# Deam0on/deepEMIA

Hardware: AMD Instinct MI355X
Metric: EM tiles/s (2048x2048, R101-FPN) (higher is better)
Workload: dtype f16x2

## Files before the change

### deepemia_amd/csrc/conv_p32.hip

```cpp
#include <utility>
#include "common.h"
#ifndef P32_ABLATE
#define P32_ABLATE 0
#endif

#ifndef P32_HEAD_DIRECT
#define P32_HEAD_DIRECT 1
#endif
#ifndef P32_SINGLE
#define P32_SINGLE 0
#endif
#ifndef P32_DEV_TILES
#define P32_DEV_TILES 0
#endif
#ifndef P32_ST_AUX
#define P32_ST_AUX 0
#endif
#ifndef P32_RES_AUX
#define P32_RES_AUX 0
#endif
#ifndef P32_A_NT
#define P32_A_NT 0
#endif
#ifndef P32_FRAG_PIPE
// ... 92 lines not shown
#pragma unroll
        for (int r = 0; r < 16; ++r)
            e[((r & 3) + 8 * (r >> 2) + 4 * (lane >> 5)) * EF + j * 32 + (lane & 31)] = row[j][r];
}
template <int TN, int EF>
__device__ __forceinline__ void write_acc16(const f32x4 (&r0)[2 * TN], const f32x4 (&r1)[2 * TN], float* e, int lane) {
#pragma unroll
    for (int j = 0; j < 2 * TN; ++j)
#pragma unroll
        for (int r = 0; r < 4; ++r) {
            e[(4 * (lane >> 4) + r) * EF + j * 16 + (lane & 15)] = r0[j][r];
            e[(16 + 4 * (lane >> 4) + r) * EF + j * 16 + (lane & 15)] = r1[j][r];
        }
}

__device__ __forceinline__ float uniform(float v) { return __int_as_float(__builtin_amdgcn_readfirstlane(__float_as_int(v))); }

struct GroupScales {
    int g0, b1, b2;
    float post0, post1, post2, resi0, resi1, resi2, sout0, sout1, sout2;
};

__device__ __forceinline__ void load_group_scale(const ConvQ& p, int gi, bool planes_out, float& post, float& resi, float& sout) {
    gi = min(gi, p.groups - 1);
    const float amax_in = p.in_meta[2 * gi], s_in = p.in_meta[2 * gi + 1];
    float amax_res = 0.f, s_res = 1.f;
    if (p.res_mode != DEMIA_RES_NONE) { amax_res = p.res_meta[2 * gi]; s_res = p.res_meta[2 * gi + 1]; }
    post = uniform(1.0f / s_in);
    resi = uniform(p.res_mode != DEMIA_RES_NONE ? 1.0f / s_res : 0.f);
    sout = uniform(planes_out ? plane_scale(amax_in * p.wbound + p.bbound + amax_res) : 1.f);
}

__device__ __forceinline__ GroupScales load_group_scales(const ConvQ& p, int m0, bool planes_out) {
    GroupScales gs;
    gs.g0 = (m0 + p.row0) / p.group_rows;
    gs.b1 = (gs.g0 + 1) * p.group_rows - p.row0;
    gs.b2 = gs.b1 + p.group_rows;
    load_group_scale(p, gs.g0, planes_out, gs.post0, gs.resi0, gs.sout0);
    load_group_scale(p, gs.g0 + 1, planes_out, gs.post1, gs.resi1, gs.sout1);
    load_group_scale(p, gs.g0 + 2, planes_out, gs.post2, gs.resi2, gs.sout2);
    return gs;
}

__device__ __forceinline__ float scale_shift(float acc, float post, float sc, float bs) { return (acc * post) * sc + bs; }
__device__ __forceinline__ void planes_item(const float4 x0, const float4 x1, float post, float res_inv, float s_out, const float (&sc)[8],
                                            const float (&bs)[8], const f16x8 ch, const f16x8 cl, float act_lo, bool sigmoid_on,
                                            f16x8& h, f16x8& l, float& vm) {
    typedef float f32x2 __attribute__((ext_vector_type(2)));
    f32x2 v2[4] = {{x0.x, x0.y}, {x0.z, x0.w}, {x1.x, x1.y}, {x1.z, x1.w}};
    float v[8];
#pragma unroll
    for (int q = 0; q < 4; ++q) {
        const f32x2 scq = {sc[2 * q], sc[2 * q + 1]}, bsq = {bs[2 * q], bs[2 * q + 1]};
        const f32x2 t = (v2[q] * post) * scq + bsq;
        v[2 * q] = t.x;
        v[2 * q + 1] = t.y;
    }
#pragma unroll
    for (int q = 0; q < 8; ++q) {
        v[q] = fmaf((float)cl[q], res_inv, fmaf((float)ch[q], res_inv, v[q]));
        v[q] = fmaxf(v[q], act_lo);
    }
    if (sigmoid_on && !(P32_ABLATE & 256)) {
#pragma unroll
        for (int q = 0; q < 8; ++q) v[q] = 1.0f / (1.0f + expf(-v[q]));
    }
    vm = 0.f;
#pragma unroll
    for (int q = 0; q < 8; q += 2) {
        vm = fmaxf(vm, fmaxf(fabsf(v[q]), fabsf(v[q + 1])));
        const f32x2 y = f32x2{v[q], v[q + 1]} * s_out;
        h[q] = (_Float16)y.x;
        h[q + 1] = (_Float16)y.y;
        l[q] = (_Float16)fmaf(-(float)h[q], 1.0f, y.x);
        l[q + 1] = (_Float16)fmaf(-(float)h[q + 1], 1.0f, y.y);
    }
}

template <int WM, int WN, int TM, int TN, bool HEAD, typename WriteRow>
__device__ __forceinline__ void p32_epilogue(const ConvQ& p, const GroupScales& gs, char* smem, WriteRow&& write_tile_row, int wm, int wn, int m0, int n0) {
    constexpr int BN = WN * TN * 32;
    const int tid = threadIdx.x, lane = tid & 63;
    constexpr int EROW = BN * 4 + 16;
    constexpr int GPR = BN / 8, RSTEP = 512 / GPR, ITEMS = WM * 32 / RSTEP;
    static_assert(512 % GPR == 0 && (WM * 32) % RSTEP == 0, "epilogue split");
    constexpr int BM_ = WM * TM * 32;
    static_assert(!HEAD || BN == 256, "the fused head needs a 256-wide tile");
    const bool planes_out = !HEAD && !p.out_f32;
    const int g0 = __builtin_amdgcn_readfirstlane(gs.g0), b1 = __builtin_amdgcn_readfirstlane(gs.b1), b2 = __builtin_amdgcn_readfirstlane(gs.b2);
    const float post0 = uniform(gs.post0), post1 = uniform(gs.post1), post2 = uniform(gs.post2);
    const float resi0 = uniform(gs.resi0), resi1 = uniform(gs.resi1), resi2 = uniform(gs.resi2);
    const float sout0 = uniform(gs.sout0), sout1 = uniform(gs.sout1), sout2 = uniform(gs.sout2);
    if (planes_out && n0 == 0 && tid == 0) {
#pragma unroll
        for (int d = 0; d < 3; ++d) {
            const int first = d == 0 ? g0 * p.group_rows - p.row0 : (d == 1 ? b1 : b2);
            if (g0 + d < p.groups && first >= m0 && first < m0 + BM_ && first < p.M)
                p.out_meta[2 * (g0 + d) + 1] = d == 0 ? sout0 : (d == 1 ? sout1 : sout2);
        }
    }
    const int g = tid % GPR, r_first = tid / GPR;
    const int co = n0 + g * 8;
    float sc[8], bs[8];
#pragma unroll
    for (int q = 0; q < 8; ++q) {
        const bool ok = (co + q) < p.Cout;
        sc[q] = (p.scale && ok) ? p.scale[co + q] : 1.0f;
        bs[q] = (p.bias && ok) ? p.bias[co + q] : 0.0f;
    }
    float vmax3[3] = {0.f, 0.f, 0.f};
    constexpr int HMAX = 4;
    float hw[HMAX][8];
    constexpr bool head_on = HEAD;
    if (head_on) {
#pragma unroll
        for (int j = 0; j < HMAX; ++j)
#pragma unroll
            for (int q = 0; q < 8; ++q) hw[j][q] = j < p.head_n ? p.head_w[j * 256 + g * 8 + q] : 0.f;
    }
    const int tile_n_ = n0 / BN;
    const bool res_on = p.res_mode != DEMIA_RES_NONE, sigmoid_on = p.act == DEMIA_ACT_SIGMOID;
    const float act_lo = p.act == DEMIA_ACT_RELU ? 0.f : -INFINITY;
    const char* resb = reinterpret_cast<const char*>(p.res) + 128;
    char* outb = reinterpret_cast<char*>(p.out) + 128;
    const long cbytes = (long)p.Cout * 4;
    const int gofs = (co >> 5) * 128 + ((co & 31) >> 3) * 16;
    auto row_of = [&](int i, int k) { const int lr = r_first + k * RSTEP; return m0 + (lr >> 5) * (TM * 32) + i * 32 + (lr & 31); };
    auto res_pix = [&](int m) -> long {
        if (p.res_mode == DEMIA_RES_SAME) return m;
        const int n = m / p.HoWo;
        const int rem = m - n * p.HoWo;
        const int ho = rem / p.Wo, wo = rem - ho * p.Wo;
        const int Hr = (p.Ho + 1) >> 1, Wr = (p.Wo + 1) >> 1;
        return ((long)n * Hr + (ho >> 1)) * Wr + (wo >> 1);
    };
    f16x8 rh[ITEMS], rl[ITEMS];
    const bool has_res = p.res_mode != DEMIA_RES_NONE && co < p.Cout;
    auto load_res = [&](int i) {
#pragma unroll
        for (int k = 0; k < ITEMS; ++k) {
            const int m = row_of(i, k);
            if (has_res && m < p.M && !(P32_ABLATE & 32)) {
                const char* rp = resb + res_pix(m) * cbytes + gofs;
                rh[k] = *reinterpret_cast<const f16x8*>(rp);
                rl[k] = *reinterpret_cast<const f16x8*>(rp + 64);
            }
        }
    };
    load_res(0);
#pragma unroll
    for (int i = 0; i < TM; ++i) {
        if (i > 0) __syncthreads();
        write_tile_row(i, reinterpret_cast<float*>(smem) + (wm * 32) * (EROW / 4) + wn * TN * 32);
        __syncthreads();
        f16x8 ch[ITEMS], cl[ITEMS];
#pragma unroll
        for (int k = 0; k < ITEMS; ++k) { ch[k] = rh[k]; cl[k] = rl[k]; }
        if (i + 1 < TM) load_res(i + 1);
        if (co < p.Cout) {
#pragma unroll
            for (int k = 0; k < ITEMS; ++k) {
                const int lr = r_first + k * RSTEP;
                const int m = row_of(i, k);
                if (m >= p.M) continue;
                const float4 x0 = *reinterpret_cast<const float4*>(smem + lr * EROW + g * 32);
                const float4 x1 = *reinterpret_cast<const float4*>(smem + lr * EROW + g * 32 + 16);
                float v[8] = {x0.x, x0.y, x0.z, x0.w, x1.x, x1.y, x1.z, x1.w};
                const int gd = (m >= b1) + (m >= b2);
// ... 27 lines not shown
#pragma unroll
                        for (int j = 0; j < HMAX; ++j)
                            if (j < p.head_n) {
                                const float z = acc_h[j] + p.head_b[j];
                                o[j] = p.head_act == DEMIA_ACT_SIGMOID ? 1.0f / (1.0f + expf(-z)) : (p.head_act == DEMIA_ACT_RELU ? fmaxf(z, 0.f) : z);
                            }
                    }
                } else if (p.out_f32) {
                    float* o = reinterpret_cast<float*>(p.out) + (long)m * p.out_ld + co;
                    if (co + 8 <= p.Cout && (p.out_ld & 3) == 0) {
                        *reinterpret_cast<float4*>(o) = make_float4(v[0], v[1], v[2], v[3]);
                        *reinterpret_cast<float4*>(o + 4) = make_float4(v[4], v[5], v[6], v[7]);
                    } else {
#pragma unroll
                        for (int q = 0; q < 8; ++q)
                            if (co + q < p.Cout) o[q] = v[q];
                    }
                } else {
                    f16x8 h, l;
                    const float s_out = gd == 0 ? sout0 : (gd == 1 ? sout1 : sout2);
                    float vm = 0.f;
#pragma unroll
                    for (int q = 0; q < 8; ++q) {
                        vm = fmaxf(vm, fabsf(v[q]));
                        const float y = v[q] * s_out;
                        h[q] = (_Float16)y;
                        l[q] = (P32_SINGLE && p.zero_low) ? (_Float16)0.f : (_Float16)(y - (float)h[q]);
                    }
                    vmax3[0] = fmaxf(vmax3[0], gd == 0 ? vm : 0.f);
                    vmax3[1] = fmaxf(vmax3[1], gd == 1 ? vm : 0.f);
                    vmax3[2] = fmaxf(vmax3[2], gd == 2 ? vm : 0.f);
                    char* o = outb + (long)m * cbytes + gofs;
                    if (P32_ABLATE & 64) {
                        asm volatile("" :: "v"(h), "v"(l), "v"(o));
                    } else {
                        *reinterpret_cast<f16x8*>(o) = h;
                        *reinterpret_cast<f16x8*>(o + 64) = l;
                    }
                }
            }
        }
    }
    if (planes_out) {
#pragma unroll
        for (int d = 0; d < 3; ++d) {
            if (d > 0 && (d == 1 ? b1 : b2) >= m0 + BM_) break;
            if (g0 + d >= p.groups) break;
            float vmax = vmax3[d];
#pragma unroll
            for (int o = 32; o > 0; o >>= 1) vmax = fmaxf(vmax, __shfl_xor(vmax, o));
            float* slot = p.out_meta + 2 * (g0 + d);
            if (lane == 0 && vmax > *reinterpret_cast<volatile const float*>(slot))
                atomicMax(reinterpret_cast<unsigned int*>(slot), __float_as_uint(vmax));
        }
    }
}

struct NoHook { __device__ __forceinline__ void operator()() const {} };
template <int WM, int WN, int TM, int TN, typename WriteRow, typename Hook = NoHook>
__device__ __forceinline__ void p32_epilogue_planes(const ConvQ& p, const GroupScales& gs, char* smem, WriteRow&& write_tile_row, int wm, int wn,
                                                    int m0, int n0, bool leader = (threadIdx.x == 0), Hook&& hook = NoHook()) {
    constexpr int BM_ = WM * TM * 32;
    const int tid = threadIdx.x, lane = tid & 63;
    constexpr int LDW = TN * 32 + 4;
    constexpr int PPW = 8 / TN, RPI = 2 * PPW, ITEMS = 32 / RPI;
    static_assert(TN == 1 || TN == 2 || TN == 4, "TN");
    char* const wsm = smem + (tid >> 6) * (32 * LDW * 4);
    const int g0 = __builtin_amdgcn_readfirstlane(gs.g0), b1 = __builtin_amdgcn_readfirstlane(gs.b1), b2 = __builtin_amdgcn_readfirstlane(gs.b2);
    const float post0 = uniform(gs.post0), post1 = uniform(gs.post1), post2 = uniform(gs.post2);
    const float resi0 = uniform(gs.resi0), resi1 = uniform(gs.resi1), resi2 = uniform(gs.resi2);
    const float sout0 = uniform(gs.sout0), sout1 = uniform(gs.sout1), sout2 = uniform(gs.sout2);
    if (n0 == 0 && leader) {
#pragma unroll
        for (int d = 0; d < 3; ++d) {
            const int first = d == 0 ? g0 * p.group_rows - p.row0 : (d == 1 ? b1 : b2);
            if (g0 + d < p.groups && first >= m0 && first < m0 + BM_ && first < p.M)
                p.out_meta[2 * (g0 + d) + 1] = d == 0 ? sout0 : (d == 1 ? sout1 : sout2);
        }
    }
    const int cj = lane & 3, rs = (lane >> 2) & 1, lg = lane >> 3;
    const int line = lg % TN;
    const int r_first = (lg / TN) * 2 + rs;
    const int co = n0 + ((wn * TN + line) * 4 + cj) * 8;
    float sc[8], bs[8];
#pragma unroll
    for (int q = 0; q < 8; ++q) {
        sc[q] = p.scale ? p.scale[co + q] : 1.0f;
        bs[q] = p.bias ? p.bias[co + q] : 0.0f;
    }
    const bool sigmoid_on = p.act == DEMIA_ACT_SIGMOID;
    const float act_lo = p.act == DEMIA_ACT_RELU ? 0.f : -INFINITY;
    const bool res_on = p.res_mode != DEMIA_RES_NONE;
    const bool single = P32_SINGLE != 0 && p.zero_low != 0;
    const __amdgpu_buffer_rsrc_t rs_out = __builtin_amdgcn_make_buffer_rsrc(p.out, 0, (int)p.out_bytes, 0x00020000);
    const __amdgpu_buffer_rsrc_t rs_res = __builtin_amdgcn_make_buffer_rsrc(const_cast<void*>(res_on ? p.res : p.out), 0, res_on ? (int)p.res_bytes : 0, 0x00020000);
    const unsigned cbytes = (unsigned)p.Cout * 4u;
    const unsigned lofs = 128u + (unsigned)((co >> 5) * 128 + (lane & 7) * 16);
    auto row_of = [&](int i, int k) { return m0 + wm * (TM * 32) + i * 32 + r_first + k * RPI; };
    auto res_off = [&](int m) -> unsigned {
        if (p.res_mode != DEMIA_RES_UP2 || (P32_ABLATE & 256)) return (unsigned)m * cbytes + lofs;
        const int n = m / p.HoWo;
        const int rem = m - n * p.HoWo;
        const int ho = rem / p.Wo, wo = rem - ho * p.Wo;
        const int Hr = (p.Ho + 1) >> 1, Wr = (p.Wo + 1) >> 1;
        return (unsigned)((n * Hr + (ho >> 1)) * Wr + (wo >> 1)) * cbytes + lofs;
    };
    auto from_below = [&](u32x4 own, u32x4 theirs) -> u32x4 {
        u32x4 r;
#pragma unroll
        for (int c = 0; c < 4; ++c) r[c] = (unsigned)__builtin_amdgcn_update_dpp((int)own[c], (int)theirs[c], 0x114, 0xf, 0xa, false);
        return r;
    };
    auto from_above = [&](u32x4 own, u32x4 theirs) -> u32x4 {
        u32x4 r;
#pragma unroll
        for (int c = 0; c < 4; ++c) r[c] = (unsigned)__builtin_amdgcn_update_dpp((int)own[c], (int)theirs[c], 0x104, 0xf, 0x5, false);
        return r;
    };
    u32x4 rh[ITEMS], rl[ITEMS];
    auto load_res = [&](int i) {
#pragma unroll
        for (int k = 0; k < ITEMS; ++k) {
            const int mp = row_of(i, k) - rs;
            if (P32_ABLATE & 32) { rh[k] = u32x4{0, 0, 0, 0}; rl[k] = rh[k]; continue; }
            rh[k] = __builtin_amdgcn_raw_buffer_load_b128(rs_res, res_off(mp), 0, P32_RES_AUX);
            rl[k] = __builtin_amdgcn_raw_buffer_load_b128(rs_res, res_off(mp + 1), 0, P32_RES_AUX);
        }
    };
    float vmax0 = 0.f, vmax1 = 0.f, vmax2 = 0.f;
    if (P32_ABLATE & 512) return;
    load_res(0);
#pragma unroll
    for (int i = 0; i < TM; ++i) {
        asm volatile("" ::: "memory");
        __builtin_amdgcn_wave_barrier();
        write_tile_row(i, reinterpret_cast<float*>(wsm));
        asm volatile("" ::: "memory");
        __builtin_amdgcn_wave_barrier();
        f16x8 ch[ITEMS], cl[ITEMS];
#pragma unroll
        for (int k = 0; k < ITEMS; ++k) {
            ch[k] = __builtin_bit_cast(f16x8, from_below(rh[k], rl[k]));
            cl[k] = __builtin_bit_cast(f16x8, from_above(rl[k], rh[k]));
        }
        if (i + 1 < TM) load_res(i + 1);
#pragma unroll
        for (int k = 0; k < ITEMS; ++k) {
            const int lr = r_first + k * RPI;
            const int m = row_of(i, k);
            const float4 x0 = *reinterpret_cast<const float4*>(wsm + lr * (LDW * 4) + (line * 4 + cj) * 32);
            const float4 x1 = *reinterpret_cast<const float4*>(wsm + lr * (LDW * 4) + (line * 4 + cj) * 32 + 16);
            const int gd = (m >= b1) + (m >= b2);
            const float post = gd == 0 ? post0 : (gd == 1 ? post1 : post2);
            const float res_inv = gd == 0 ? resi0 : (gd == 1 ? resi1 : resi2);
            const float s_out = gd == 0 ? sout0 : (gd == 1 ? sout1 : sout2);
            f16x8 h, l;
            float vm;
            planes_item(x0, x1, post, res_inv, s_out, sc, bs, ch[k], cl[k], act_lo, sigmoid_on, h, l, vm);
            if (single) l = f16x8{0, 0, 0, 0, 0, 0, 0, 0};
            vm = m < p.M ? vm : 0.f;
            vmax0 = fmaxf(vmax0, gd == 0 ? vm : 0.f);
            vmax1 = fmaxf(vmax1, gd == 1 ? vm : 0.f);
            vmax2 = fmaxf(vmax2, gd == 2 ? vm : 0.f);
            const u32x4 hu = __builtin_bit_cast(u32x4, h), lu = __builtin_bit_cast(u32x4, l);
            const u32x4 d0 = from_below(hu, lu);
            const u32x4 d1 = from_above(lu, hu);
            const unsigned off = (unsigned)(m - rs) * cbytes + lofs;
            if (P32_ABLATE & 64) {
                asm volatile("" :: "v"(d0), "v"(d1), "v"(off));
            } else {
                __builtin_amdgcn_raw_buffer_store_b128(d0, rs_out, off, 0, P32_ST_AUX);
                __builtin_amdgcn_raw_buffer_store_b128(d1, rs_out, off + cbytes, 0, P32_ST_AUX);
            }
            hook();
        }
    }
#pragma unroll
    for (int d = 0; d < 3; ++d) {
        if (d > 0 && (d == 1 ? b1 : b2) >= m0 + BM_) break;
        if (g0 + d >= p.groups) break;
        float vmax = d == 0 ? vmax0 : (d == 1 ? vmax1 : vmax2);
#pragma unroll
        for (int o = 32; o > 0; o >>= 1) vmax = fmaxf(vmax, __shfl_xor(vmax, o));
        float* slot = p.out_meta + 2 * (g0 + d);
        if (lane == 0 && vmax > *reinterpret_cast<volatile const float*>(slot))
            atomicMax(reinterpret_cast<unsigned int*>(slot), __float_as_uint(vmax));
    }
}

template <int WM, int WN, int TM, int TN, int HN>
__device__ __forceinline__ void p32_epilogue_head_direct(const ConvQ& p, const GroupScales& gs, char* smem, const f32x4 (&acc16)[2 * TM][2 * TN],
                                                         int wm, int wn, int m0, int n0) {
    constexpr int BM = WM * TM * 32, BN = WN * TN * 32;
    static_assert(BN == 256, "the fused head needs a 256-wide tile");
    const int tid = threadIdx.x, lane = tid & 63, c16 = lane & 15, rq = lane >> 4;
    const int b1 = __builtin_amdgcn_readfirstlane(gs.b1), b2 = __builtin_amdgcn_readfirstlane(gs.b2);
    const float post0 = uniform(gs.post0), post1 = uniform(gs.post1), post2 = uniform(gs.post2);
    float sc[2 * TN], bs[2 * TN], hw[HN][2 * TN];
#pragma unroll
    for (int jn = 0; jn < 2 * TN; ++jn) {
        const int cl = wn * TN * 32 + jn * 16 + c16;
        sc[jn] = p.scale ? p.scale[n0 + cl] : 1.0f;
        bs[jn] = p.bias ? p.bias[n0 + cl] : 0.0f;
#pragma unroll
        for (int j = 0; j < HN; ++j) hw[j][jn] = j < p.head_n ? p.head_w[j * 256 + cl] : 0.f;
    }
    const float act_lo = p.act == DEMIA_ACT_RELU ? 0.f : -INFINITY;
    float* part = reinterpret_cast<float*>(smem);
#pragma unroll
    for (int i = 0; i < 2 * TM; ++i) {
#pragma unroll
        for (int r = 0; r < 4; ++r) {
            const int row = wm * TM * 32 + i * 16 + rq * 4 + r;
            const int m = m0 + row;
            const int gd = (m >= b1) + (m >= b2);
            const float post = gd == 0 ? post0 : (gd == 1 ? post1 : post2);
            float a[HN];
#pragma unroll
            for (int j = 0; j < HN; ++j) a[j] = 0.f;
#pragma unroll
            for (int jn = 0; jn < 2 * TN; ++jn) {
                const float v = fmaxf((acc16[i][jn][r] * post) * sc[jn] + bs[jn], act_lo);
#pragma unroll
                for (int j = 0; j < HN; ++j) a[j] = fmaf(v, hw[j][jn], a[j]);
            }
#pragma unroll
            for (int j = 0; j < HN; ++j) {
                a[j] += __int_as_float(__builtin_amdgcn_update_dpp(0, __float_as_int(a[j]), 0x128, 0xf, 0xf, false));
                a[j] += __int_as_float(__builtin_amdgcn_update_dpp(0, __float_as_int(a[j]), 0x124, 0xf, 0xf, false));
                a[j] += __int_as_float(__builtin_amdgcn_update_dpp(0, __float_as_int(a[j]), 0x122, 0xf, 0xf, false));
// ... 52 lines not shown
    const int line = lg % TN;
    const int r_first = (lg / TN) * 2 + rs;
    const int cgrp = wn * TN + line;
    const int co = (cgrp * 4 + cj) * 8;
    float sc[8], bs[8];
#pragma unroll
    for (int q = 0; q < 8; ++q) {
        sc[q] = p.scale ? p.scale[co + q] : 1.0f;
        bs[q] = p.bias ? p.bias[co + q] : 0.0f;
    }
    const bool sigmoid_on = p.act == DEMIA_ACT_SIGMOID;
    const float act_lo = p.act == DEMIA_ACT_RELU ? 0.f : -INFINITY;
    const f16x8 zero8 = {0, 0, 0, 0, 0, 0, 0, 0};
    const int r16 = lane & 15, kq = lane >> 4, fsw = (r16 >> 1) & 7;
    const bool c_ok = r16 < p.hp_cout;
    const float hsc = (p.hp_scale && c_ok) ? p.hp_scale[r16] : 1.0f;
    const float hbs = (p.hp_bias && c_ok) ? p.hp_bias[r16] : 0.0f;
#pragma unroll
    for (int i = 0; i < TM; ++i) {
        asm volatile("" ::: "memory");
        __builtin_amdgcn_wave_barrier();
        write_tile_row(i, reinterpret_cast<float*>(wsm));
        asm volatile("" ::: "memory");
        __builtin_amdgcn_wave_barrier();
        f16x8 h[ITEMS], l[ITEMS];
#pragma unroll
        for (int k = 0; k < ITEMS; ++k) {
            const int lr = r_first + k * RPI;
            const int m = m0 + wm * (TM * 32) + i * 32 + lr;
            const float4 x0 = *reinterpret_cast<const float4*>(wsm + lr * (LDW * 4) + (line * 4 + cj) * 32);
            const float4 x1 = *reinterpret_cast<const float4*>(wsm + lr * (LDW * 4) + (line * 4 + cj) * 32 + 16);
            const int gd = (m >= b1) + (m >= b2);
            const float post = gd == 0 ? post0 : (gd == 1 ? post1 : post2);
            const float s_out = gd == 0 ? sout0 : (gd == 1 ? sout1 : sout2);
            float vm;
            planes_item(x0, x1, post, 0.f, s_out, sc, bs, zero8, zero8, act_lo, sigmoid_on, h[k], l[k], vm);
        }
        if (i > 0) __syncthreads();
#pragma unroll
        for (int k = 0; k < ITEMS; ++k) {
            const int R = wm * 32 + r_first + k * RPI, sw = (R >> 1) & 7;
            char* ln = img + (cgrp * ROWS + R) * 128;
            *reinterpret_cast<f16x8*>(ln + ((cj ^ sw) * 16)) = h[k];
            *reinterpret_cast<f16x8*>(ln + (((4 + cj) ^ sw) * 16)) = l[k];
        }
        if (i == 0) {
#pragma unroll
            for (int q = 0; q < 2; ++q) {
                const int c = tid + q * 512, g = c >> 7, row = (c >> 3) & 15, ck = c & 7;
                *reinterpret_cast<u32x4*>(wimg + g * 2048 + row * 128 + ((ck ^ ((row >> 1) & 7)) * 16)) = wreg[q];
            }
        }
        __syncthreads();
        if (wave < ROWS / 16) {
            f32x4 c = {0.f, 0.f, 0.f, 0.f};
#pragma unroll
            for (int g = 0; g < 8; ++g) {
                const char* ab = img + (g * ROWS + wave * 16 + r16) * 128;
                const char* bb = wimg + g * 2048 + r16 * 128;
                const f16x8 ah = *reinterpret_cast<const f16x8*>(ab + ((kq ^ fsw) * 16));
                const f16x8 al = *reinterpret_cast<const f16x8*>(ab + (((4 + kq) ^ fsw) * 16));
                const f16x8 bh = *reinterpret_cast<const f16x8*>(bb + ((kq ^ fsw) * 16));
                const f16x8 bl = *reinterpret_cast<const f16x8*>(bb + (((4 + kq) ^ fsw) * 16));
                c = __builtin_amdgcn_mfma_f32_16x16x32_f16(ah, bl, c, 0, 0, 0);
                c = __builtin_amdgcn_mfma_f32_16x16x32_f16(al, bh, c, 0, 0, 0);
                c = __builtin_amdgcn_mfma_f32_16x16x32_f16(ah, bh, c, 0, 0, 0);
            }
#pragma unroll
            for (int r = 0; r < 4; ++r) {
                const int R = wave * 16 + kq * 4 + r;
                const int m = m0 + (R >> 5) * (TM * 32) + i * 32 + (R & 31);
                const int gd = (m >= b1) + (m >= b2);
                const float ipost = gd == 0 ? ipost0 : (gd == 1 ? ipost1 : ipost2);
                const float z = fmaxf(scale_shift(c[r], ipost, hsc, hbs), -INFINITY);
                if (m < p.M && c_ok) p.head_out[(long)m * p.head_ld + r16] = z;
            }
        }
    }
}

constexpr int EPI_GENERIC = 0, EPI_PLANES = 1, EPI_HEAD = 2, EPI_HEAD_PLANES = 3;

template <int WM, int WN, int TM, int TN, bool M16 = true, int EPI = EPI_PLANES, int NST = 2, bool HK = false>
__global__ __launch_bounds__(WM * WN * 64, WM * WN == 8 ? 2 : 1) void conv_p32_kernel(const ConvQ p) {
    static_assert(NST == 2 || NST == 3, "two or three LDS stages");
    static_assert(!HK || (P32_SINGLE && M16 && NST == 2), "HK is a variant of the single-plane 16x16x32 kernel");
    static_assert(WM * WN == 8 || (WM * WN == 4 && EPI == EPI_PLANES), "eight waves, or four (planes epilogue only)");
    constexpr int NW = WM * WN;
    constexpr int BM = WM * TM * 32, BN = WN * TN * 32;
    constexpr int STAGE = (BM + BN) * 128;
    constexpr int NIA = BM / 8, NIB = BN / 8;

    extern __shared__ __attribute__((aligned(16))) char smem[];
    const int tid = threadIdx.x, lane = tid & 63;
    const int wave = __builtin_amdgcn_readfirstlane(tid >> 6);
    const int wm = wave / WN, wn = wave % WN;
    const int swz = xcd_remap(blockIdx.x, p.nwg);
    const int tile_n = swz % p.ntn, tile_m = swz / p.ntn;
    const int m0 = tile_m * BM, n0 = tile_n * BN;
#if P32_DEV_TILES
    if (p.stagger_ticks > 0) {
        const int b = blockIdx.x;
        const bool late = p.resident > 256 ? (b >= p.resident / 2 && b < p.resident) : (b < p.resident && ((b >> 3) & 1));
        if (late) {
            const unsigned long long t0 = __builtin_amdgcn_s_memrealtime();
            while (__builtin_amdgcn_s_memrealtime() - t0 < (unsigned long long)p.stagger_ticks) __builtin_amdgcn_s_sleep(32);
        }
    }
#endif

    const i32x4 rsrc_a = make_rsrc(p.in, p.in_bytes), rsrc_b = make_rsrc(p.w, p.w_bytes);
    const unsigned lds0 = (unsigned)(__SIZE_TYPE__)((lds_void*)smem);

    constexpr int QA = (NIA + NW - 1) / NW, QB = NIB / NW;
    constexpr bool A_EVEN = NIA % NW == 0;
    static_assert(NIB % NW == 0, "tile width is a multiple of 64");
    unsigned a_off[QA], a_msk[QA], b_off[QB];
#pragma unroll
    for (int q = 0; q < QA; ++q) {
        const int row = (wave + NW * q) * 8 + (lane >> 3);
        const int csw = (lane & 7) ^ ((row >> 1) & 7);
        const int m = m0 + row;
        const bool vm = m < p.M && row < BM;
        const int mm = vm ? m : 0;
        const int n = mm / p.HoWo;
        const int rem = mm - n * p.HoWo;
        const int ho = rem / p.Wo, wo = rem - ho * p.Wo;
        const int hi0 = ho * p.stride - p.pad, wi0 = wo * p.stride - p.pad;
        const long pix = ((long)n * p.H + hi0) * p.W + wi0;
        a_off[q] = (unsigned)(128 + pix * (long)(p.Cin * 4) + (HK ? (csw >> 2) * 128 + (csw & 3) * 16 : csw * 16));
        unsigned mk = 0;
        for (int t = 0, th = 0, tw = 0; t < p.taps; ++t) {
            if (vm && (unsigned)(hi0 + th) < (unsigned)p.H && (unsigned)(wi0 + tw) < (unsigned)p.W) mk |= 1u << t;
            if (++tw == p.KW) { tw = 0; ++th; }
        }
        a_msk[q] = mk;
    }
#pragma unroll
    for (int q = 0; q < QB; ++q) {
        const int row = (wave + NW * q) * 8 + (lane >> 3);
        const int csw = (lane & 7) ^ ((row >> 1) & 7);
        const int co = n0 + row;
        b_off[q] = (unsigned)(((co >> 6) * p.ksteps) * 8192 + (co & 63) * 128 + (HK ? (csw >> 2) * (p.taps * 8192) + (csw & 3) * 16 : csw * 16));
    }
    int tap = 0, kw = 0, tstep = 0;
    unsigned sdelta = 0, srow = 0, sgrp = 0;
    const bool a_nt = P32_A_NT && p.taps == 1 && p.ntn == 1;
    auto issue = [&](int st, int tp, unsigned sd, unsigned bd) {
        const unsigned sbase = __builtin_amdgcn_readfirstlane(lds0 + st * STAGE + wave * 1024);
        const bool first = bd < 2 * 8192u;
#pragma unroll
        for (int q = 0; q < QA; ++q) {
            if ((P32_ABLATE & 1) && !first) break;
            if (!A_EVEN && q == QA - 1 && wave + NW * q >= NIA) break;
            const bool ok = (a_msk[q] >> tp) & 1u;
            const unsigned vo = ok ? a_off[q] + sd : (a_off[q] & 0x70u);
            if (P32_A_NT && a_nt) dma16_nt(rsrc_a, sbase + q * (NW * 1024), vo, 0u);
            else dma16(rsrc_a, sbase + q * (NW * 1024), vo, 0u);
        }
#pragma unroll
        for (int q = 0; q < QB; ++q) {
            if ((P32_ABLATE & 2) && !first) break;
            dma16(rsrc_b, sbase + BM * 128 + q * (NW * 1024), b_off[q], bd);
        }
    };
    const unsigned pixb = (unsigned)(p.Cin * 4), rowb = (unsigned)(p.W * p.Cin * 4);
#define P32_ADVANCE()                                                                   \
    do {                                                                                \
        ++tstep;                                                                        \
        if (++tap == p.taps) { tap = 0; kw = 0; srow = 0; sgrp += HK ? 256u : 128u; sdelta = sgrp; if (HK) tstep += p.taps; } \
// ... 192 lines not shown
#pragma unroll
        for (int kk = 0; kk < 2; ++kk) {
            f16x8 bh[TN], bl[TN];
#pragma unroll
            for (int j = 0; j < TN; ++j) {
                bh[j] = *reinterpret_cast<const f16x8*>(sb + fb[kk] + j * 4096);
                bl[j] = *reinterpret_cast<const f16x8*>(sb + fb[2 + kk] + j * 4096);
            }
#pragma unroll
            for (int i = 0; i < TM; ++i) {
                const f16x8 ah = *reinterpret_cast<const f16x8*>(sb + fa[kk] + i * 4096);
                const f16x8 al = *reinterpret_cast<const f16x8*>(sb + fa[2 + kk] + i * 4096);
#pragma unroll
                for (int j = 0; j < TN; ++j) {
                    f32x16 c = acc[i][j];
                    if (P32_ABLATE & 4) {
                        asm volatile("" :: "v"(ah), "v"(al), "v"(bh[j]), "v"(bl[j]));
                        continue;
                    }
                    c = __builtin_amdgcn_mfma_f32_32x32x16_f16(ah, bl[j], c, 0, 0, 0);
                    c = __builtin_amdgcn_mfma_f32_32x32x16_f16(al, bh[j], c, 0, 0, 0);
                    c = __builtin_amdgcn_mfma_f32_32x32x16_f16(ah, bh[j], c, 0, 0, 0);
                    acc[i][j] = c;
                }
            }
        }
    };

    constexpr int N_LAST = QB + QA, N_LAST_SHORT = QB + QA - 1;
    const bool short_wave = !A_EVEN && wave + NW * (QA - 1) >= NIA;
    auto wait_all_but_last_issue = [&]() {
        if (short_wave) asm volatile("s_waitcnt vmcnt(%0)" ::"n"(N_LAST_SHORT) : "memory");
        else asm volatile("s_waitcnt vmcnt(%0)" ::"n"(N_LAST) : "memory");
    };
    issue(0, tap, sdelta, 0u);
    P32_ADVANCE();
    bool two_ahead = false;
    if (NST == 3 && p.kloop > 1 && !(P32_ABLATE & 128)) {
        issue(1, tap, sdelta, (unsigned)tstep * 8192u);
        P32_ADVANCE();
        two_ahead = true;
    }
    constexpr bool HEAD = EPI == EPI_HEAD;
    const GroupScales gs = load_group_scales(p, m0, !HEAD && !p.out_f32);
    if (two_ahead) wait_all_but_last_issue();
    else asm volatile("s_waitcnt vmcnt(0)" ::: "memory");
    __builtin_amdgcn_s_barrier();
    int st = 0;
    for (int t = 0; t < ((P32_ABLATE & 128) ? 1 : p.kloop); ++t) {
        const int st_issue = NST == 2 ? (st ^ 1) : (st == 0 ? 2 : st - 1);
        const bool more = t + NST - 1 < p.kloop;
        if (more) {
            issue(st_issue, tap, sdelta, (unsigned)tstep * 8192u);
            P32_ADVANCE();
        }
        compute(st);
        if (NST == 3 && more) {
            wait_all_but_last_issue();
            asm volatile("s_waitcnt lgkmcnt(0)\n\ts_barrier" ::: "memory");
        } else if (!BARRIER_IN_COMPUTE) {
            asm volatile("s_waitcnt vmcnt(0) lgkmcnt(0)\n\ts_barrier" ::: "memory");
        }
        st = NST == 2 ? (st ^ 1) : (st == 2 ? 0 : st + 1);
    }
#undef P32_ADVANCE

    if constexpr ((P32_ABLATE & 2048) != 0 && M16) {
#pragma unroll
        for (int i = 0; i < 2 * TM; ++i)
#pragma unroll
            for (int j = 0; j < 2 * TN; ++j) asm volatile("" :: "v"(acc16[i][j]));
        return;
    }
    if constexpr (EPI == EPI_HEAD_PLANES) {
        static_assert(M16, "the fused 1x1 layer rides on the 16x16x32 kernel");
        p32_epilogue_head_planes<WM, WN, TM, TN>(p, gs, smem, [&](int i, float* e) { write_acc16<TN, TN * 32 + 4>(acc16[2 * i], acc16[2 * i + 1], e, lane); }, wm, wn, m0);
    } else if constexpr (EPI == EPI_PLANES) {
        if constexpr (M16) {
            p32_epilogue_planes<WM, WN, TM, TN>(p, gs, smem, [&](int i, float* e) { write_acc16<TN, TN * 32 + 4>(acc16[2 * i], acc16[2 * i + 1], e, lane); }, wm, wn, m0, n0);
        } else {
            p32_epilogue_planes<WM, WN, TM, TN>(p, gs, smem, [&](int i, float* e) { write_acc32<TN, TN * 32 + 4>(acc[i], e, lane); }, wm, wn, m0, n0);
        }
    } else if constexpr (M16 && HEAD && P32_HEAD_DIRECT) {
        if (p.act != DEMIA_ACT_SIGMOID && p.head_n <= 2)
            p32_epilogue_head_direct<WM, WN, TM, TN, 2>(p, gs, smem, acc16, wm, wn, m0, n0);
        else
            p32_epilogue<WM, WN, TM, TN, HEAD>(p, gs, smem, [&](int i, float* e) { write_acc16<TN, BN + 4>(acc16[2 * i], acc16[2 * i + 1], e, lane); }, wm, wn, m0, n0);
    } else if constexpr (M16) {
        p32_epilogue<WM, WN, TM, TN, HEAD>(p, gs, smem, [&](int i, float* e) { write_acc16<TN, BN + 4>(acc16[2 * i], acc16[2 * i + 1], e, lane); }, wm, wn, m0, n0);
    } else {
        p32_epilogue<WM, WN, TM, TN, HEAD>(p, gs, smem, [&](int i, float* e) { write_acc32<TN, BN + 4>(acc[i], e, lane); }, wm, wn, m0, n0);
    }
}

#if P32_DEV_TILES
#include "conv_p32_dev.inc"
#endif

template <int WM, int WN, int TM, int TN, bool M16 = true, int EPI = EPI_PLANES, int NST = 2, bool HK = false>
int launch_q_(ConvQ p, hipStream_t st) {
    constexpr int BM = WM * TM * 32, BN = WN * TN * 32;
    constexpr int stages = NST * (BM + BN) * 128, image = EPI == EPI_HEAD_PLANES ? HeadPlanesLds<WM, WN, TM, TN>::BYTES
                                                         : (EPI == EPI_PLANES ? WM * WN * 32 * (TN * 128 + 16) : WM * 32 * (BN * 4 + 16));
    static_assert(stages <= 160 * 1024 && image <= 160 * 1024, "LDS");
    constexpr int smem = stages > image ? stages : image;
    p.ntn = p.CoutPad / BN;
    p.nwg = p.ntn * cdiv(p.M, BM);
    p.resident = 256 * (160 * 1024 / smem >= 2 ? 2 : 1);
    p.kloop = HK ? p.ksteps / 2 : p.ksteps;
    auto k = conv_p32_kernel<WM, WN, TM, TN, M16, EPI, NST, HK>;
    static bool attr_done = false;
    if (!attr_done) {
        (void)hipFuncSetAttribute(reinterpret_cast<const void*>(k), hipFuncAttributeMaxDynamicSharedMemorySize, smem);
        attr_done = true;
    }
    hipLaunchKernelGGL(k, dim3(p.nwg), dim3(WM * WN * 64), smem, st, p);
    DEMIA_CHECK_LAUNCH("conv_p32_kernel");
    return DEMIA_OK;
}
template <int WM, int WN, int TM, int TN, bool M16 = true, int EPI = EPI_PLANES, int NST = 2>
int launch_q(ConvQ p, hipStream_t st) {
#if P32_SINGLE
    if constexpr (M16 && NST == 2) {
        if (p.Cin % 64 == 0 && !p.no_hk) return launch_q_<WM, WN, TM, TN, M16, EPI, NST, true>(p, st);
    }
#endif
    return launch_q_<WM, WN, TM, TN, M16, EPI, NST, false>(p, st);
}

struct TileCfg { int id, bm, bn; };
constexpr TileCfg kTiles[] = {{1, 256, 256}, {2, 128, 256}, {4, 192, 256}, {12, 160, 256}, {13, 224, 256}, {6, 256, 128}, {7, 128, 128}, {9, 256, 64}, {11, 128, 64}};

inline double predict_us(const TileCfg& c, long M, int cout_pad, int ksteps, bool residual) {
    const long tiles = (long)cdiv(M, c.bm) * (cout_pad / c.bn);
    const int smem = 2 * (c.bm + c.bn) * 128;
    const int occ = 160 * 1024 / smem >= 2 ? 2 : 1;
    const double area = (double)c.bm * c.bn / 65536.0;
    const double step = 2.0 * area * (1.0 + 0.2 * (1.0 - area));
    const double edge = 6.0 + 6.0 * area * (residual ? 1.5 : 1.0);
    if (occ == 1) return (double)((tiles + 255) / 256) * (ksteps * step + edge);
    return (double)((tiles + 511) / 512) * (2.0 * ksteps * step + 2.0 * 0.5 * edge);
}

inline int choose_tile(long M, int cout_pad, int ksteps, bool residual, bool need256 = false) {
#if P32_SINGLE
    if (cout_pad % 256 == 0 && (long)cdiv(M, 256) * (cout_pad / 256) >= 512) return 1;
#endif
    int best = 0;
    double best_t = 1e30;
    for (const TileCfg& c : kTiles) {
        if (cout_pad % c.bn || (need256 && c.bn != 256)) continue;
        const double t = predict_us(c, M, cout_pad, ksteps, residual);
        if (t < best_t) { best_t = t; best = c.id; }
    }
    return best;
}

}

#if P32_SINGLE
extern "C" int demia_conv2d_p32_single(const demia_conv_p32_desc* d, void* stream) {
#else
extern "C" int demia_conv2d_p32_single(const demia_conv_p32_desc* d, void* stream);
extern "C" int demia_conv2d_p32(const demia_conv_p32_desc* d, void* stream) {
    if (d && d->single) return demia_conv2d_p32_single(d, stream);
#endif
    DEMIA_REQUIRE(d && d->in && d->in_meta && d->w && (d->out || d->head_n > 0 || d->head_planes), "null pointer");
    DEMIA_REQUIRE(d->out_f32 || d->out_meta || d->head_n > 0 || d->head_planes, "P32 output needs out_meta");
    DEMIA_REQUIRE(d->Cin > 0 && d->Cin % 32 == 0, "Cin must be a multiple of 32");
    DEMIA_REQUIRE(d->CoutPad >= d->Cout && d->CoutPad % 64 == 0, "CoutPad must be a multiple of 64");
    DEMIA_REQUIRE(d->out_f32 || d->Cout % 32 == 0, "P32 output needs Cout % 32 == 0");
    DEMIA_REQUIRE(d->KH > 0 && d->KW > 0 && d->KH * d->KW <= 32 && d->stride > 0 && d->pad >= 0, "kernel geometry");
    DEMIA_REQUIRE(d->Ho == (d->H + 2 * d->pad - d->KH) / d->stride + 1, "Ho");
    DEMIA_REQUIRE(d->Wo == (d->W + 2 * d->pad - d->KW) / d->stride + 1, "Wo");
    DEMIA_REQUIRE(d->res_mode == DEMIA_RES_NONE || (d->residual && d->res_meta), "residual pointer");
    DEMIA_REQUIRE((long)d->N * d->Ho * d->Wo < (1L << 31), "M overflow");
    const long in_bytes = 128 + (long)d->N * d->H * d->W * d->Cin * 4;
    DEMIA_REQUIRE(in_bytes < (1L << 32), "input planes must stay below 4 GiB");
    const long w_bytes = (long)d->CoutPad * d->KH * d->KW * d->Cin * 4;
    DEMIA_REQUIRE(w_bytes < (1L << 31), "weight planes must stay below 2 GiB");
    ConvQ p;
    p.in = d->in; p.in_meta = d->in_meta; p.w = d->w; p.scale = d->scale; p.bias = d->bias;
    p.res = d->residual; p.res_meta = d->res_meta; p.out = d->out; p.out_meta = d->out_meta;
    p.wbound = d->wbound; p.bbound = d->bbound;
    p.N = d->N; p.H = d->H; p.W = d->W; p.Cin = d->Cin; p.Ho = d->Ho; p.Wo = d->Wo; p.Cout = d->Cout; p.CoutPad = d->CoutPad;
    p.KH = d->KH; p.KW = d->KW; p.stride = d->stride; p.pad = d->pad;
    p.act = d->act; p.res_mode = d->res_mode; p.out_f32 = d->out_f32;
    p.out_ld = d->out_ld > 0 ? d->out_ld : d->Cout;
    DEMIA_REQUIRE(p.out_ld >= d->Cout, "out_ld");
    p.M = d->N * d->Ho * d->Wo;
    p.HoWo = d->Ho * d->Wo;
    p.taps = d->KH * d->KW;
    p.ksteps = p.taps * (d->Cin / 32);
    p.in_bytes = (unsigned)in_bytes; p.w_bytes = (unsigned)w_bytes;
    p.ntn = p.nwg = 0;
    p.zero_low = d->single == 2;
    {
        static const char* env = getenv("DEMIA_P32_NO_HK");
        p.no_hk = (env && env[0] == '1') ? 1 : 0;
    }
    p.kloop = 0;
    p.resident = 256;
    p.groups = d->groups > 1 ? d->groups : 1;
    p.group_rows = p.groups > 1 ? d->group_rows : (1 << 29);
    p.row0 = p.groups > 1 ? d->row0 : 0;
    DEMIA_REQUIRE(p.groups == 1 || (d->group_rows >= 128 && d->row0 >= 0 && ((long)p.M + d->row0 + d->group_rows - 1) / d->group_rows <= p.groups),
                  "scale groups: group_rows >= 128 and the rows of this call must fall inside `groups` groups");
    p.head_w = d->head_w; p.head_b = d->head_b; p.head_out = d->head_out; p.head_n = d->head_n; p.head_ld = d->head_ld; p.head_act = d->head_act;
    if (d->head_n > 0) {
        DEMIA_REQUIRE(d->head_n <= 4 && d->head_w && d->head_b && d->head_out && d->head_ld >= d->head_n, "fused head: at most 4 rows, pointers, head_ld");
        DEMIA_REQUIRE(d->CoutPad % 256 == 0 && d->Cout == d->CoutPad && !d->out_f32, "fused head needs Cout % 256 == 0 and a planes layer");
    }
    p.hp_w = d->head_planes; p.hp_scale = d->head_scale; p.hp_bias = d->head_bias; p.hp_cout = d->head_cout;
    if (d->head_planes) {
#if P32_SINGLE
        DEMIA_REQUIRE(false, "fused 1x1 layer (head_planes): not in the single-plane build");
#endif
        DEMIA_REQUIRE(d->head_n == 0 && d->head_out && d->head_cout >= 1 && d->head_cout <= 16 && d->head_ld >= d->head_cout,
                      "fused 1x1 layer: head_n == 0, head_out, 1 <= head_cout <= 16, head_ld >= head_cout");
        DEMIA_REQUIRE(d->Cout == 256 && d->CoutPad == 256 && !d->out_f32 && d->res_mode == DEMIA_RES_NONE,
                      "fused 1x1 layer needs a planes layer of exactly 256 channels without residual");
    }
    p.stagger_ticks = 0;
#if P32_DEV_TILES
    {
        static const char* env = getenv("DEMIA_P32_STAGGER_US");
        p.stagger_ticks = env ? atoi(env) * 100 : 0;
    }
#endif
    if (p.M == 0) return DEMIA_OK;
    hipStream_t st = reinterpret_cast<hipStream_t>(stream);
    int tile = d->tile_hint ? d->tile_hint : choose_tile(p.M, d->CoutPad, p.ksteps, d->res_mode != DEMIA_RES_NONE, d->head_n > 0 || d->head_planes);
    const bool n256 = d->CoutPad % 256 == 0, n128 = d->CoutPad % 128 == 0;
#if !P32_SINGLE
    if (d->head_planes) {
        if (!d->tile_hint && cdiv(p.M, 128) <= 128) tile = 15;
        switch (tile) {
            case 1: return launch_q<2, 4, 4, 2, true, EPI_HEAD_PLANES>(p, st);
            case 2: return launch_q<2, 4, 2, 2, true, EPI_HEAD_PLANES>(p, st);
            case 15: return launch_q<1, 8, 2, 1, true, EPI_HEAD_PLANES>(p, st);
            default: return launch_q<1, 8, 6, 1, true, EPI_HEAD_PLANES>(p, st);
        }
    }
#endif
    if (d->head_n > 0) {
        switch (tile) {
            case 1: return launch_q<2, 4, 4, 2, true, EPI_HEAD>(p, st);
            case 2: return launch_q<2, 4, 2, 2, true, EPI_HEAD>(p, st);
            default: return launch_q<1, 8, 6, 1, true, EPI_HEAD>(p, st);
        }
    }
    const int tile_bn = (tile == 9 || tile == 10 || tile == 11 || tile == 49) ? 64 : ((tile >= 6 && tile <= 8) || tile == 26 ? 128 : 256);
    const long out_bytes = 128 + (long)p.M * d->Cout * 4;
    long res_bytes = 0;
    if (d->res_mode == DEMIA_RES_SAME) res_bytes = out_bytes;
    if (d->res_mode == DEMIA_RES_UP2) res_bytes = 128 + (long)d->N * ((d->Ho + 1) / 2) * ((d->Wo + 1) / 2) * d->Cout * 4;
    const bool planes = !d->out_f32 && d->Cout % tile_bn == 0 && out_bytes < (1L << 32) - 512 && res_bytes < (1L << 32) - 512 &&
                        (long)(p.M + 256) * d->Cout * 4 + 256 < (1L << 32);
    p.out_bytes = (unsigned)out_bytes; p.res_bytes = (unsigned)res_bytes;
#if !P32_SINGLE && P32_DEV_TILES
    if (tile == 60) {
        DEMIA_REQUIRE(!d->out_f32 && n128 && d->Cout % 128 == 0 && d->KH == 1 && d->KW == 1 && d->stride == 1 && d->pad == 0 &&
                      d->res_mode != DEMIA_RES_UP2 && out_bytes < (1L << 32) - 512 && res_bytes < (1L << 32) - 512 &&
                      (long)(p.M + 256) * d->Cout * 4 + 256 < (1L << 32),
                      "tile 60 (ping-pong) takes 1x1 stride-1 planes layers with Cout % 128 == 0, no nearest-2x residual, buffers below 4 GiB");
        return launch_pp1x1(p, st);
    }
#endif
    if (!planes) {
        if (tile != 7 && tile != 9 && tile != 10 && tile != 11 && tile != 21 && tile != 22 && tile != 26) tile = n128 ? 7 : 11;
        switch (tile) {
            case 7: DEMIA_REQUIRE(n128, "tile needs CoutPad % 128 == 0"); return launch_q<4, 2, 1, 2, true, EPI_GENERIC>(p, st);
            case 9: return launch_q<8, 1, 1, 2, true, EPI_GENERIC>(p, st);
            case 10: return launch_q<4, 2, 2, 1, true, EPI_GENERIC>(p, st);
            case 11: return launch_q<4, 2, 1, 1, true, EPI_GENERIC>(p, st);
            default: break;
        }
    }
    switch (tile) {
        case 1: DEMIA_REQUIRE(n256, "tile needs CoutPad % 256 == 0"); return launch_q<2, 4, 4, 2>(p, st);
        case 2: DEMIA_REQUIRE(n256, "tile needs CoutPad % 256 == 0"); return launch_q<2, 4, 2, 2>(p, st);
        case 4: DEMIA_REQUIRE(n256, "tile needs CoutPad % 256 == 0"); return launch_q<1, 8, 6, 1>(p, st);
        case 6: DEMIA_REQUIRE(n128, "tile needs CoutPad % 128 == 0"); return launch_q<4, 2, 2, 2>(p, st);
        case 7: DEMIA_REQUIRE(n128, "tile needs CoutPad % 128 == 0"); return launch_q<4, 2, 1, 2>(p, st);
        case 9: return launch_q<8, 1, 1, 2>(p, st);
        case 11: return launch_q<4, 2, 1, 1>(p, st);
        case 12: DEMIA_REQUIRE(n256, "tile needs CoutPad % 256 == 0"); return launch_q<1, 8, 5, 1>(p, st);
        case 13: DEMIA_REQUIRE(n256, "tile needs CoutPad % 256 == 0"); return launch_q<1, 8, 7, 1>(p, st);
#if P32_DEV_TILES
        case 3: DEMIA_REQUIRE(n256, "tile needs CoutPad % 256 == 0"); return launch_q<1, 8, 8, 1>(p, st);
        case 5: DEMIA_REQUIRE(n256, "tile needs CoutPad % 256 == 0"); return launch_q<1, 8, 4, 1>(p, st);
        case 8: DEMIA_REQUIRE(n128, "tile needs CoutPad % 128 == 0"); return launch_q<2, 4, 2, 1>(p, st);
        case 10: return launch_q<4, 2, 2, 1>(p, st);
        case 14: DEMIA_REQUIRE(n256, "tile needs CoutPad % 256 == 0"); return launch_q<2, 4, 3, 2>(p, st);
        case 42: DEMIA_REQUIRE(n256, "tile needs CoutPad % 256 == 0"); return launch_q<2, 4, 2, 2, true, EPI_PLANES, 3>(p, st);
        case 52: DEMIA_REQUIRE(n256, "tile needs CoutPad % 256 == 0"); return launch_q<1, 8, 5, 1, true, EPI_PLANES, 3>(p, st);
        case 49: return launch_q<8, 1, 1, 2, true, EPI_PLANES, 3>(p, st);
        case 31: DEMIA_REQUIRE(n256, "tile needs CoutPad % 256 == 0"); return launch_q<2, 4, 4, 2, false>(p, st);
        case 34: DEMIA_REQUIRE(n256, "tile needs CoutPad % 256 == 0"); return launch_q<1, 8, 6, 1, false>(p, st);
        case 21: DEMIA_REQUIRE(n256, "tile needs CoutPad % 256 == 0"); return launch_pp<4, 2>(p, st);
        case 22: DEMIA_REQUIRE(n256, "tile needs CoutPad % 256 == 0"); return launch_pp<2, 2>(p, st);
        case 26: DEMIA_REQUIRE(n128, "tile needs CoutPad % 128 == 0"); return launch_pp<4, 1>(p, st);
#endif
        default: DEMIA_REQUIRE(false, "tile_hint");
    }
    return DEMIA_EINVAL;
}
```

Measured before the change: 748.6.

## Add sixteen-wave conv tiles for fused head and deep-K layers

Allows 16-wave (1024-thread) workgroups in the p32 conv kernel. Tile 1 now dispatches to a 4x4-wave layout for the fused head and a 2x8-wave layout for layers with many K steps. The epilogue thread split is generalised to the actual thread count. The planes epilogue gets a rolling two-slot residual prefetch and defers the scale/bias loads so fewer registers stay live with 16 waves. Launch bounds now scale with wave count. The extra waves are meant to hide latency in the main loop, at the cost of tighter per-thread register budgets and possible spills.

```diff
diff --git a/deepemia_amd/csrc/conv_p32.hip b/deepemia_amd/csrc/conv_p32.hip
--- a/deepemia_amd/csrc/conv_p32.hip
+++ b/deepemia_amd/csrc/conv_p32.hip
@@ -198,8 +198,9 @@
     constexpr int BN = WN * TN * 32;
     const int tid = threadIdx.x, lane = tid & 63;
     constexpr int EROW = BN * 4 + 16;
-    constexpr int GPR = BN / 8, RSTEP = 512 / GPR, ITEMS = WM * 32 / RSTEP;
-    static_assert(512 % GPR == 0 && (WM * 32) % RSTEP == 0, "epilogue split");
+    constexpr int NT = WM * WN * 64;
+    constexpr int GPR = BN / 8, RSTEP = NT / GPR, ITEMS = WM * 32 / RSTEP;
+    static_assert(NT % GPR == 0 && (WM * 32) % RSTEP == 0, "epilogue split");
     constexpr int BM_ = WM * TM * 32;
     static_assert(!HEAD || BN == 256, "the fused head needs a 256-wide tile");
     const bool planes_out = !HEAD && !p.out_f32;
@@ -393,11 +394,15 @@
     const int line = lg % TN;
     const int r_first = (lg / TN) * 2 + rs;
     const int co = n0 + ((wn * TN + line) * 4 + cj) * 8;
+    constexpr bool TIGHT = WM * WN == 16 && TN == 2;
+    constexpr int RES_AHEAD = 2;
     float sc[8], bs[8];
-#pragma unroll
-    for (int q = 0; q < 8; ++q) {
-        sc[q] = p.scale ? p.scale[co + q] : 1.0f;
-        bs[q] = p.bias ? p.bias[co + q] : 0.0f;
+    if constexpr (!TIGHT) {
+#pragma unroll
+        for (int q = 0; q < 8; ++q) {
+            sc[q] = p.scale ? p.scale[co + q] : 1.0f;
+            bs[q] = p.bias ? p.bias[co + q] : 0.0f;
+        }
     }
     const bool sigmoid_on = p.act == DEMIA_ACT_SIGMOID;
     const float act_lo = p.act == DEMIA_ACT_RELU ? 0.f : -INFINITY;
@@ -429,18 +434,24 @@
         return r;
     };
     u32x4 rh[ITEMS], rl[ITEMS];
+    auto load_res_item = [&](int i, int k, int slot) {
+        const int mp = row_of(i, k) - rs;
+        if (P32_ABLATE & 32) { rh[slot] = u32x4{0, 0, 0, 0}; rl[slot] = rh[slot]; return; }
+        rh[slot] = __builtin_amdgcn_raw_buffer_load_b128(rs_res, res_off(mp), 0, P32_RES_AUX);
+        rl[slot] = __builtin_amdgcn_raw_buffer_load_b128(rs_res, res_off(mp + 1), 0, P32_RES_AUX);
+    };
     auto load_res = [&](int i) {
 #pragma unroll
-        for (int k = 0; k < ITEMS; ++k) {
-            const int mp = row_of(i, k) - rs;
-            if (P32_ABLATE & 32) { rh[k] = u32x4{0, 0, 0, 0}; rl[k] = rh[k]; continue; }
-            rh[k] = __builtin_amdgcn_raw_buffer_load_b128(rs_res, res_off(mp), 0, P32_RES_AUX);
-            rl[k] = __builtin_amdgcn_raw_buffer_load_b128(rs_res, res_off(mp + 1), 0, P32_RES_AUX);
-        }
+        for (int k = 0; k < ITEMS; ++k) load_res_item(i, k, k);
     };
     float vmax0 = 0.f, vmax1 = 0.f, vmax2 = 0.f;
     if (P32_ABLATE & 512) return;
-    load_res(0);
+    if constexpr (TIGHT) {
+#pragma unroll
+        for (int j = 0; j < RES_AHEAD; ++j) load_res_item(j / ITEMS, j % ITEMS, j);
+    } else {
+        load_res(0);
+    }
 #pragma unroll
     for (int i = 0; i < TM; ++i) {
         asm volatile("" ::: "memory");
@@ -448,15 +459,32 @@
         write_tile_row(i, reinterpret_cast<float*>(wsm));
         asm volatile("" ::: "memory");
         __builtin_amdgcn_wave_barrier();
+        if constexpr (TIGHT) {
+            if (i == 0) {
+#pragma unroll
+                for (int q = 0; q < 8; ++q) {
+                    sc[q] = p.scale ? p.scale[co + q] : 1.0f;
+                    bs[q] = p.bias ? p.bias[co + q] : 0.0f;
+                }
+            }
+        }
         f16x8 ch[ITEMS], cl[ITEMS];
+        auto exchange = [&](int k, int slot) {
+            ch[k] = __builtin_bit_cast(f16x8, from_below(rh[slot], rl[slot]));
+            cl[k] = __builtin_bit_cast(f16x8, from_above(rl[slot], rh[slot]));
+        };
+        if constexpr (!TIGHT) {
+#pragma unroll
+            for (int k = 0; k < ITEMS; ++k) exchange(k, k);
+            if (i + 1 < TM) load_res(i + 1);
+        }
 #pragma unroll
         for (int k = 0; k < ITEMS; ++k) {
-            ch[k] = __builtin_bit_cast(f16x8, from_below(rh[k], rl[k]));
-            cl[k] = __builtin_bit_cast(f16x8, from_above(rl[k], rh[k]));
-        }
-        if (i + 1 < TM) load_res(i + 1);
-#pragma unroll
-        for (int k = 0; k < ITEMS; ++k) {
+            if constexpr (TIGHT) {
+                const int j = i * ITEMS + k, slot = j % RES_AHEAD;
+                exchange(k, slot);
+                if (j + RES_AHEAD < TM * ITEMS) load_res_item((j + RES_AHEAD) / ITEMS, (j + RES_AHEAD) % ITEMS, slot);
+            }
             const int lr = r_first + k * RPI;
             const int m = row_of(i, k);
             const float4 x0 = *reinterpret_cast<const float4*>(wsm + lr * (LDW * 4) + (line * 4 + cj) * 32);
@@ -675,10 +703,11 @@
 constexpr int EPI_GENERIC = 0, EPI_PLANES = 1, EPI_HEAD = 2, EPI_HEAD_PLANES = 3;
 
 template <int WM, int WN, int TM, int TN, bool M16 = true, int EPI = EPI_PLANES, int NST = 2, bool HK = false>
-__global__ __launch_bounds__(WM * WN * 64, WM * WN == 8 ? 2 : 1) void conv_p32_kernel(const ConvQ p) {
+__global__ __launch_bounds__(WM * WN * 64, WM * WN / 4) void conv_p32_kernel(const ConvQ p) {
     static_assert(NST == 2 || NST == 3, "two or three LDS stages");
     static_assert(!HK || (P32_SINGLE && M16 && NST == 2), "HK is a variant of the single-plane 16x16x32 kernel");
-    static_assert(WM * WN == 8 || (WM * WN == 4 && EPI == EPI_PLANES), "eight waves, or four (planes epilogue only)");
+    static_assert(WM * WN == 8 || (WM * WN == 4 && EPI == EPI_PLANES) || (WM * WN == 16 && EPI != EPI_HEAD_PLANES),
+                  "eight waves, four (planes epilogue only) or sixteen (not the fused 1x1 layer)");
     constexpr int NW = WM * WN;
     constexpr int BM = WM * TM * 32, BN = WN * TN * 32;
     constexpr int STAGE = (BM + BN) * 128;
@@ -1037,7 +1066,9 @@
             p32_epilogue_planes<WM, WN, TM, TN>(p, gs, smem, [&](int i, float* e) { write_acc32<TN, TN * 32 + 4>(acc[i], e, lane); }, wm, wn, m0, n0);
         }
     } else if constexpr (M16 && HEAD && P32_HEAD_DIRECT) {
-        if (p.act != DEMIA_ACT_SIGMOID && p.head_n <= 2)
+        if constexpr (NW == 16)
+            p32_epilogue_head_direct<WM, WN, TM, TN, 2>(p, gs, smem, acc16, wm, wn, m0, n0);
+        else if (p.act != DEMIA_ACT_SIGMOID && p.head_n <= 2)
             p32_epilogue_head_direct<WM, WN, TM, TN, 2>(p, gs, smem, acc16, wm, wn, m0, n0);
         else
             p32_epilogue<WM, WN, TM, TN, HEAD>(p, gs, smem, [&](int i, float* e) { write_acc16<TN, BN + 4>(acc16[2 * i], acc16[2 * i + 1], e, lane); }, wm, wn, m0, n0);
@@ -1199,9 +1230,14 @@
     }
 #endif
     if (d->head_n > 0) {
+        const bool head16 = !P32_SINGLE && P32_HEAD_DIRECT && d->act != DEMIA_ACT_SIGMOID && d->head_n <= 2;
         switch (tile) {
-            case 1: return launch_q<2, 4, 4, 2, true, EPI_HEAD>(p, st);
+            case 1: return head16 ? launch_q<4, 4, 2, 2, true, EPI_HEAD>(p, st) : launch_q<2, 4, 4, 2, true, EPI_HEAD>(p, st);
             case 2: return launch_q<2, 4, 2, 2, true, EPI_HEAD>(p, st);
+#if P32_DEV_TILES
+            case 61: DEMIA_REQUIRE(head16, "sixteen-wave fused head: ReLU / no activation, at most 2 head rows"); return launch_q<4, 4, 2, 2, true, EPI_HEAD>(p, st);
+            case 65: return launch_q<2, 4, 4, 2, true, EPI_HEAD>(p, st);
+#endif
             default: return launch_q<1, 8, 6, 1, true, EPI_HEAD>(p, st);
         }
     }
@@ -1232,8 +1268,9 @@
             default: break;
         }
     }
+    const bool waves16 = !P32_SINGLE && p.ksteps >= 72;
     switch (tile) {
-        case 1: DEMIA_REQUIRE(n256, "tile needs CoutPad % 256 == 0"); return launch_q<2, 4, 4, 2>(p, st);
+        case 1: DEMIA_REQUIRE(n256, "tile needs CoutPad % 256 == 0"); return waves16 ? launch_q<2, 8, 4, 1>(p, st) : launch_q<2, 4, 4, 2>(p, st);
         case 2: DEMIA_REQUIRE(n256, "tile needs CoutPad % 256 == 0"); return launch_q<2, 4, 2, 2>(p, st);
         case 4: DEMIA_REQUIRE(n256, "tile needs CoutPad % 256 == 0"); return launch_q<1, 8, 6, 1>(p, st);
         case 6: DEMIA_REQUIRE(n128, "tile needs CoutPad % 128 == 0"); return launch_q<4, 2, 2, 2>(p, st);
@@ -1253,6 +1290,11 @@
         case 49: return launch_q<8, 1, 1, 2, true, EPI_PLANES, 3>(p, st);
         case 31: DEMIA_REQUIRE(n256, "tile needs CoutPad % 256 == 0"); return launch_q<2, 4, 4, 2, false>(p, st);
         case 34: DEMIA_REQUIRE(n256, "tile needs CoutPad % 256 == 0"); return launch_q<1, 8, 6, 1, false>(p, st);
+        case 65: DEMIA_REQUIRE(n256, "tile needs CoutPad % 256 == 0"); return launch_q<2, 4, 4, 2>(p, st);
+        case 61: DEMIA_REQUIRE(n256, "tile needs CoutPad % 256 == 0"); return launch_q<4, 4, 2, 2>(p, st);
+        case 62: DEMIA_REQUIRE(n256, "tile needs CoutPad % 256 == 0"); return launch_q<2, 8, 4, 1>(p, st);
+        case 63: DEMIA_REQUIRE(n256, "tile needs CoutPad % 256 == 0"); return launch_q<4, 4, 1, 2>(p, st);
+        case 64: DEMIA_REQUIRE(n256, "tile needs CoutPad % 256 == 0"); return launch_q<2, 8, 2, 1>(p, st);
         case 21: DEMIA_REQUIRE(n256, "tile needs CoutPad % 256 == 0"); return launch_pp<4, 2>(p, st);
         case 22: DEMIA_REQUIRE(n256, "tile needs CoutPad % 256 == 0"); return launch_pp<2, 2>(p, st);
         case 26: DEMIA_REQUIRE(n128, "tile needs CoutPad % 128 == 0"); return launch_pp<4, 1>(p, st);
```

After: 759.0, median of 6. +1.4%, better.
